# chinmay5/vit_ae_plus_plus

Measured on AMD Instinct MI355X. Metric: pretrain volumes/sec (96^3x4ch, mask 0.75) at 1/2/4/8 MI355X + recon-loss parity, higher is better.
Workload: dtype bf16; 1 GPU; ViT-B/16^3 contrastive MAE full optimisation step (fwd+loss+bwd+grad-norm+AdamW), synthetic BraTS-shape 96^3x4ch, batch 4/GPU, mask 0.75 (BASELINE config 2); global_batch=4, parallelism=dp1, rccl_ranks=1, hip_graph=True, weights=product initialize_weights, seed 0

## Files before the change

vit_ae_plus_plus_amd/csrc/gemm_bt.hpp:

```cpp
#pragma once
#include <cstdlib>
#include <type_traits>
#include "glds_gemm.hpp"

namespace vglds {

using K0 = std::integral_constant<int, 0>; using K1 = std::integral_constant<int, 1>;
using K2 = std::integral_constant<int, 2>; using K3 = std::integral_constant<int, 3>;

__device__ __forceinline__ void wg_barrier() {
    __builtin_amdgcn_sched_barrier(0);
    __builtin_amdgcn_s_barrier();
    __builtin_amdgcn_sched_barrier(0);
}


template <int S, int PT> __device__ __forceinline__ void wait_tiles(const int fly) {
    if (S >= 5 && fly >= 3) wait_vmcnt<(S >= 5 ? 3 : 1) * PT>();
    else if (S >= 4 && fly >= 2) wait_vmcnt<(S >= 4 ? 2 : 1) * PT>();
    else if (fly >= 1) wait_vmcnt<PT>();
    else wait_vmcnt<0>();
}

static inline bool bt_k_ranges(const int K, const int min_tiles, int& splits, int& kps) {
// ... 67 lines not shown
#pragma unroll
            for (int e = 0; e < 4; ++e) v[e] += bias4[e];
            f32x4 axv = {0.f, 0.f, 0.f, 0.f};
            if (need_aux) {
                if constexpr (AUX16) {
                    const bf16x4 h = ax16[pb * LB + q];
                    axv = f32x4{(float)h[0], (float)h[1], (float)h[2], (float)h[3]};
                } else {
                    axv = ax[pb * LB + q];
                }
            }
            if (epi == VITAE_EPI_GELU) {
                f32x4 y, dy;
                if (p.exact) {
#pragma unroll
                    for (int e = 0; e < 4; ++e) { float ye, de; gelu_erf_both(v[e], ye, de); y[e] = ye; dy[e] = de; }
                } else {
                    gelu_fast4(v, y, dy);
                }
                const f32x4 sv = p.auxd ? dy : v;
                if (ok) {
                    if constexpr (AUX16) {
                        bf16x4 h;
#pragma unroll
                        for (int e = 0; e < 4; ++e) h[e] = (__bf16)sv[e];
                        *reinterpret_cast<bf16x4*>(reinterpret_cast<__bf16*>(p.aux) + m * ldaux + n) = h;
                    } else {
                        *reinterpret_cast<f32x4*>(p.aux + m * ldaux + n) = sv;
                    }
                }
                v = y;
            } else if (epi == VITAE_EPI_DGELU) {
                f32x4 g = axv;
                if (!p.auxd) {
                    if (p.exact) {
#pragma unroll
                        for (int e = 0; e < 4; ++e) g[e] = gelu_erf_grad(axv[e]);
                    } else {
                        g = gelu_fast_grad4(axv);
                    }
                }
#pragma unroll
                for (int e = 0; e < 4; ++e) v[e] *= g[e];
            } else if (epi == VITAE_EPI_RELU_MASK) {
#pragma unroll
                for (int e = 0; e < 4; ++e) v[e] = axv[e] > 0.f ? v[e] : 0.f;
            } else if (epi == VITAE_EPI_RELU) {
#pragma unroll
                for (int e = 0; e < 4; ++e) v[e] = fmaxf(v[e], 0.f);
            }
            if (has_res) {
#pragma unroll
                for (int e = 0; e < 4; ++e) v[e] += rs[pb * LB + q][e];
            }
            if (acc_c) {
#pragma unroll
                for (int e = 0; e < 4; ++e) v[e] += co[pb * LB + q][e];
            }
            if (ok) {
                if (p.C) *reinterpret_cast<f32x4*>(p.C + m * ldc + n) = v;
                if (p.C16) {
                    bf16x4 v16;
#pragma unroll
                    for (int e = 0; e < 4; ++e) v16[e] = (__bf16)v[e];
                    *reinterpret_cast<bf16x4*>(p.C16 + m * ldc16 + n) = v16;
                }
                if (p.out_colsum) {
#pragma unroll
                    for (int e = 0; e < 4; ++e) csum[e] += v[e];
                }
                if (p.sqacc) sqs += (v[0] * v[0] + v[1] * v[1]) + (v[2] * v[2] + v[3] * v[3]);
            }
        }
    }
}

__device__ __forceinline__ int bt_epilogue_kind(const GArgs& p) {
    const bool res = p.residual != nullptr, accc = p.C && p.accumulate;
    if (p.epi == VITAE_EPI_NONE) return res && accc ? 7 : res ? 1 : accc ? 2 : 0;
    if (res || accc) return 7;
    return p.epi == VITAE_EPI_GELU ? 3 : p.epi == VITAE_EPI_DGELU ? 4 : p.epi == VITAE_EPI_RELU_MASK ? 5 : p.epi == VITAE_EPI_RELU ? 6 : 7;
}

template <int FM, int FN>
__device__ __forceinline__ void bt_wave_epilogue(const GArgs& p, int kind, int mb, int nb, const float* Tw, int lane, float& sqs, const f32x4 bias4,
                                                 f32x4& csum, const bool defer_colsum) {
    constexpr int LPR = 8 * FN;
    const bool full = mb + 32 * FM <= p.M && nb + 32 * FN <= p.N;
#define VITAE_BT_ROWS(E)                                                                       \
    case E:                                                                                    \
        if (full) bt_wave_rows<FM, FN, E, true, false>(p, mb, nb, Tw, lane, sqs, csum, bias4);  \
        else bt_wave_rows<FM, FN, E, false, false>(p, mb, nb, Tw, lane, sqs, csum, bias4);      \
        break;
#define VITAE_BT_ROWS_AUX(E)                                                                   \
    case E:                                                                                    \
        if (p.aux16) {                                                                         \
            if (full) bt_wave_rows<FM, FN, E, true, true>(p, mb, nb, Tw, lane, sqs, csum, bias4);  \
            else bt_wave_rows<FM, FN, E, false, true>(p, mb, nb, Tw, lane, sqs, csum, bias4);      \
        } else {                                                                               \
            if (full) bt_wave_rows<FM, FN, E, true, false>(p, mb, nb, Tw, lane, sqs, csum, bias4); \
            else bt_wave_rows<FM, FN, E, false, false>(p, mb, nb, Tw, lane, sqs, csum, bias4);     \
        }                                                                                      \
        break;
    switch (kind) {
        VITAE_BT_ROWS(0) VITAE_BT_ROWS(1) VITAE_BT_ROWS(2) VITAE_BT_ROWS_AUX(3) VITAE_BT_ROWS_AUX(4) VITAE_BT_ROWS_AUX(5) VITAE_BT_ROWS(6)
        default:
            if (p.aux16) bt_wave_rows<FM, FN, 7, false, true>(p, mb, nb, Tw, lane, sqs, csum, bias4);
            else bt_wave_rows<FM, FN, 7, false, false>(p, mb, nb, Tw, lane, sqs, csum, bias4);
            break;
    }
#undef VITAE_BT_ROWS
#undef VITAE_BT_ROWS_AUX
    if (defer_colsum) return;
    if (p.out_colsum) {
#pragma unroll
        for (int e = 0; e < 4; ++e)
#pragma unroll
            for (int d = LPR; d < 64; d <<= 1) csum[e] += __shfl_xor(csum[e], d, 64);
        const int n = nb + 4 * (lane % LPR);
        if (lane < LPR && n < p.N) {
#pragma unroll
            for (int e = 0; e < 4; ++e) atomicAdd(p.out_colsum + n + e, csum[e]);
        }
    }
}

template <int FM, int FN, int NACC>
__device__ __forceinline__ void bt_park_quadrant(const f32x16 (&acc)[NACC][FM * FN], int lane, float* Tw) {
    constexpr int S = 32 * FN;
    const int l31 = lane & 31, hi = lane >> 5;
#pragma unroll
    for (int fm = 0; fm < FM; ++fm)
#pragma unroll
        for (int fn = 0; fn < FN; ++fn)
#pragma unroll
            for (int r = 0; r < 16; ++r) {
                float v = acc[0][fm * FN + fn][r];
                if (NACC == 2) v += acc[NACC - 1][fm * FN + fn][r];
                Tw[(fm * 32 + crow(r, hi)) * S + fn * 32 + l31] = v;
            }
}

template <int BM, int BN, int WM, int WN, int NACC, class Stamp>
__device__ __forceinline__ void bt_tail(const GArgs& p, f32x16 (&acc)[2][2][NACC][BtCfg<BM, BN, WM, WN>::FM * BtCfg<BM, BN, WM, WN>::FN],
                                        unsigned char* smem, const int m0, const int n0, const int tm, const int tn, const int zid,
                                        const int wave, const int lane, Stamp stamp) {
    using Cf = BtCfg<BM, BN, WM, WN>;
    constexpr int NW = Cf::NW, HM = Cf::HM, HN = Cf::HN, FM = Cf::FM, FN = Cf::FN, NF = FM * FN;
    const int wm = wave / WN, wn = wave % WN;
    constexpr int TW = 32 * FM * 32 * FN;
    static_assert(NW * TW * 4 + 64 <= Cf::SMEM, "wave-private staging (+ the norm share of each wave) fits the operand stages");
    float* Tw = reinterpret_cast<float*>(smem) + wave * TW;
    float sqs = 0.f;
    const int kind = bt_epilogue_kind(p);
    if constexpr (BM * BN < 256 * 256) if (p.splits > 1) {
        constexpr int NT = 64 * NW, GROUPS = 4 * NF * 4;
        const int tile = p.tile0 + tm * p.tiles_n + tn;
        float* part = p.ws + VITAE_GLDS_TICKETS + (long)tile * p.splits * (NT * GROUPS * 4);
        const __amdgpu_buffer_rsrc_t rs = __builtin_amdgcn_make_buffer_rsrc(part, 0, p.splits * (NT * GROUPS * 16), 0x00020000);
        typedef unsigned u32x4 __attribute__((ext_vector_type(4)));
        const int toff = (int)threadIdx.x * 16;
        if constexpr (NACC == 2) {
#pragma unroll
            for (int a = 0; a < 2; ++a)
#pragma unroll
                for (int b = 0; b < 2; ++b)
#pragma unroll
                    for (int f = 0; f < NF; ++f)
#pragma unroll
                        for (int i = 0; i < 16; ++i) acc[a][b][0][f][i] += acc[a][b][NACC - 1][f][i];
        }
#pragma unroll
        for (int a = 0; a < 2; ++a)
#pragma unroll
            for (int b = 0; b < 2; ++b)
#pragma unroll
                for (int f = 0; f < NF; ++f)
#pragma unroll
                    for (int g = 0; g < 4; ++g) {
                        f32x4 v;
#pragma unroll
                        for (int e = 0; e < 4; ++e) v[e] = acc[a][b][0][f][4 * g + e];
                        const int grp = ((a * 2 + b) * NF + f) * 4 + g;
                        __builtin_amdgcn_raw_buffer_store_b128(__builtin_bit_cast(u32x4, v), rs, (zid * GROUPS + grp) * (NT * 16) + toff, 0, 16);
// ... 140 lines not shown
```

vit_ae_plus_plus_amd/csrc/gemm_glds.hip:

```cpp
#include <cstdlib>
#include "common.hpp"
#include "glds_tiles.hpp"
#include "glds_gemm.hpp"
#include "vitae_hip.h"

namespace {

using namespace vglds;

long long* g_gemm_dbg = nullptr;
double* g_wgrad_sqacc = nullptr;
int g_wgrad_sq_mask = 0, g_wgrad_sq_stride = 0;
static inline void set_sq(vglds::GArgs& p) { p.sqacc = g_wgrad_sqacc; p.sq_mask = g_wgrad_sq_mask; p.sq_stride = g_wgrad_sq_stride; }

struct EpiPre { f32x4 bias, res[4]; bool have; };

template <int BM, int BN, int NW>
__device__ __forceinline__ void epilogue_prefetch(const GArgs& p, int m0, int n0, EpiPre& e) {
    constexpr int NT = 64 * NW, CG = BN / 4, RPP = NT / CG, PASSES = BM / RPP;
    e.have = false;
    if constexpr (BM == 64 && BN == 64 && NW == 4) {
        static_assert(PASSES == 4, "prefetch geometry");
        if (!p.vec_epi) return;
        e.have = true;
// ... 462 lines not shown
    if (wave == 0 && n < N) {
        const f32x4 t = (red[0][lane] + red[1][lane]) + (red[2][lane] + red[3][lane]);
#pragma unroll
        for (int e = 0; e < 4; ++e) atomicAdd(out + n + e, t[e]);
    }
}

inline void launch_colsum_bf16(const void* dy16, float* out, int M, int N, hipStream_t st) {
    const int gx = cdiv(N, 256);
    constexpr int tgt = 320;
    int rpw = cdiv(cdiv(M, cdiv(tgt, gx)), 4);
    if (rpw < 4) rpw = 4;
    hipLaunchKernelGGL(colsum_bf16_kernel, dim3(gx, cdiv(M, 4 * rpw)), dim3(256), 0, st, reinterpret_cast<const __bf16*>(dy16), out, M, N, rpw);
}

struct Tile { int bm, bn, id; };

inline int vec_epilogue_ok(const GArgs& p) {
    if (p.N & 3) return 0;
    auto ok = [](const void* ptr, long ld, int align) { return !ptr || (!(ld & 3) && !((uintptr_t)ptr & (align - 1))); };
    return ok(p.C, p.ldc, 16) && ok(p.C16, p.ldc16, 8) && ok(p.aux, p.ldaux, 16) && ok(p.residual, p.ldr, 16) && ok(p.bias, 0, 16);
}

inline int xcd_by_rows(int M, int N) { return M > N; }

inline Tile pick_tile(int M, int N) {
    constexpr int wide_min = 400;
    if (N >= 128 && (long)cdiv(M, 64) * cdiv(N, 128) >= wide_min) return {64, 128, 1};
    return {64, 64, 0};
}

int g_bt_mode = env_int("VITAE_BT_TILE", -1);

struct BtPlan { int tile, split; double clocks; };

inline int old_split_rule(int M, int N, int K) {
    constexpr int min_kt = 8, target = 384;
    const Tile t = pick_tile(M, N);
    const long tiles = (long)cdiv(M, t.bm) * cdiv(N, t.bn);
    if (tiles >= target / 2 || tiles > VITAE_GLDS_TICKETS) return 1;
    long s = (target + tiles - 1) / tiles;
    const long max_by_k = K / (BK * min_kt);
    if (s > max_by_k) s = max_by_k;
    if (s > 32) s = 32;
    return s < 1 ? 1 : (int)s;
}

inline double est_64row(int M, int N, int K, bool allow_split, bool wgrad_form) {
    const Tile t = pick_tile(M, N);
    const int s = allow_split ? old_split_rule(M, N, K) : 1;
    const double nk = (double)K / BK / s, wgs = (double)cdiv(M, t.bm) * cdiv(N, t.bn) * s;
    const double c = t.id == 1 ? 3800 + 1250 * nk : 5100 + (wgrad_form ? 650 : 400) * nk;
    const double lat = 8000 + (t.id == 1 ? 1000 : 760) * nk + (s > 1 ? 7000 : 0);
    const double thr = wgs * c / 256;
    return thr > lat ? thr : lat;
}

inline BtPlan bt_plan(int M, int N, int K, int a_kc, int b_kc, bool allow_split, long cap = -1, bool allow_ws64 = true, int only = -1) {
    BtPlan best{-1, 1, 1e30};
    if (g_bt_mode == -2 || K < 2 * BK || (K % BK) || (!a_kc && b_kc) || (N & 3)) return best;
    const int nkt = K / BK;
    constexpr double ws_kt = 800.0;
    constexpr int ws_min_rows = 2048;
    constexpr int ws_min_rows_fwd = 800;
    constexpr int ws_long_k = 8192;
    constexpr double ws_kt_w = 900.0;
    constexpr double ws_fix = 14000.0;
    constexpr double ws64_kt_w = 650.0;
    constexpr double bt_fix0 = 9000.0, bt_fix1 = 4000.0;
    constexpr double wsw_kt = 1350.0;
    for (int id : {0, 3, 4, 5, 6, 7}) {
        if (only >= 0 && id != only) continue;
        if (id == 7 && g_bt_mode != 7 && only != 7) continue;
        if (id == 6 && (a_kc || b_kc)) continue;
        if (id == 5 && g_bt_mode != 5 && !allow_ws64) continue;
        if (g_bt_mode >= 0 && id != g_bt_mode) continue;
        if (id == 4 && g_bt_mode < 0 && (a_kc ? M : K) < ((a_kc && b_kc) ? ws_min_rows_fwd : ws_min_rows) && K < ws_long_k) continue;
        if (id == 6 && g_bt_mode < 0 && K < ws_min_rows && K < ws_long_k && (long)M * N < (1L << 22)) continue;
        int bm, bn;
        bt_tile_dims(id, bm, bn);
        const bool forced = g_bt_mode >= 0;
        if (!forced && (M < bm / 2 || N < bn / 2)) continue;
        const long tiles = (long)cdiv(M, bm) * cdiv(N, bn);
        const int fsplit = ENV_INT_ONCE("VITAE_BT_SPLIT", 0);
        for (int s = 1; s <= (id >= 3 && allow_split ? (id == 6 ? 4 : 8) : 1); ++s) {
            if (forced && fsplit > 0 && s != fsplit) continue;
            const int kps = cdiv(cdiv(K, s), BK) * BK;
            if (cdiv(K, kps) != s || kps < (forced ? 2 : 4) * BK || K - (s - 1) * kps < 2 * BK) continue;
            if (s > 1 && (tiles > VITAE_GLDS_TICKETS || (cap >= 0 && VITAE_GLDS_TICKETS + tiles * s * bm * bn > cap))) continue;
            const double wgs = (double)tiles * s, slots = id == 3 ? 512 : 256;
            const double rounds = (double)cdiv((long)wgs, (long)slots);
            const double nk = (double)nkt / s;
            const double per = id == 0 ? 3000 + ((!a_kc && !b_kc) ? 4300 : 2950) * nk + 14500
                             : id == 6 ? ws_fix + 4000 + wsw_kt * nk + (s > 1 ? 9000 + 4000 * s : 0)
                             : id == 4 ? ws_fix + ((!a_kc && !b_kc) ? ws_kt_w : ws_kt) * nk + (s > 1 ? 6000 + 2200 * s : 0)
                                       : 4500 + 1800 * nk + 7500 + (s > 1 ? bt_fix0 + bt_fix1 * s : 0);
            double clk = rounds * per;
            if (id == 7) {
                const double over = wgs > 256 ? (wgs - 256) / 256 : 0, kt = ((!a_kc && !b_kc && wgs >= 512) ? ws64_kt_w : 420) * 1.5;
                const double lat = (7500 + kt * nk + (s > 1 ? 3000 + 1000 * s : 0)) * (1 + 0.2 * over), thr = wgs * (4000 + kt * nk) / 256;
                clk = lat > thr ? lat : thr;
                if (nkt >= 128) clk *= 1.25;
            }
            if (id == 5) {
                const double over = wgs > 256 ? (wgs - 256) / 256 : 0, kt64 = (!a_kc && !b_kc && wgs >= 512) ? ws64_kt_w : 420;
                const double lat = (6500 + kt64 * nk + (s > 1 ? 3000 + 1000 * s : 0)) * (1 + 0.2 * over), thr = wgs * (3000 + kt64 * nk) / 256;
                clk = lat > thr ? lat : thr;
                if (nkt >= 128) clk *= 1.25;
            }
            if (clk < best.clocks) best = BtPlan{id, s, clk};
        }
    }
    if (best.tile < 0 || g_bt_mode >= 0 || only >= 0) return best;
    if (best.clocks >= 0.92 * est_64row(M, N, K, allow_split, !a_kc && !b_kc) * (nkt >= 128 ? 1.25 : 1.0)) return BtPlan{-1, 1, 0.0};
    return best;
}

template <int BM1, int BN1>
void launch_pair(int id2, dim3 grid, hipStream_t st, const GArgs& p1, const GArgs& p2, int nb1) {
    dim3 block(256);
    if (id2 == 0) hipLaunchKernelGGL((gemm_glds_pair_kernel<BM1, BN1, 64, 64>), grid, block, 0, st, p1, p2, nb1);
    else hipLaunchKernelGGL((gemm_glds_pair_kernel<BM1, BN1, 64, 128>), grid, block, 0, st, p1, p2, nb1);
}

}

extern "C" int vitae_gemm_glds_set_bt_tile(int mode) {
    if (mode < -2 || mode > 7 || mode == 1 || mode == 2) return VITAE_ERR_INVALID_ARG;
    g_bt_mode = mode;
    return VITAE_OK;
}

extern "C" int vitae_gemm_glds_bt_choice(int a_kcontig, int b_kcontig, int M, int N, int K) { return bt_plan(M, N, K, a_kcontig, b_kcontig, true).tile; }

extern "C" int vitae_gemm_glds_pick_split_k(int M, int N, int K) {
    const BtPlan bp = bt_plan(M, N, K, 1, 1, true);
    if (bp.tile >= 0) return bp.split;
    return old_split_rule(M, N, K);
}

extern "C" int vitae_gemm_glds_pick_split_k_form(int a_kcontig, int b_kcontig, int M, int N, int K) {
    const BtPlan bp = bt_plan(M, N, K, a_kcontig, b_kcontig, true);
    if (bp.tile >= 0) return bp.split;
    return old_split_rule(M, N, K);
}

extern "C" long vitae_gemm_glds_ws_floats(int M, int N, int split_k) {
    if (split_k <= 1) return 0;
    const Tile t = pick_tile(M, N);
    const long small = (long)cdiv(M, t.bm) * cdiv(N, t.bn) * t.bm * t.bn, big = (long)cdiv(M, 128) * cdiv(N, 128) * 128 * 128;
    const long wide = (long)cdiv(M, 128) * cdiv(N, 256) * 128 * 256;
    long m = small > big ? small : big;
    if (wide > m) m = wide;
    return VITAE_GLDS_TICKETS + m * split_k;
}

static int gemm_glds_launch(int a_kcontig, int b_kcontig, const void* A16, long lda, const void* B16, long ldb,
                            float* C, long ldc, void* C16, long ldc16, int M, int N, int K, const float* bias,
                            const float* residual, long ldr, int epi, float* aux, long ldaux, int accumulate,
                            int split_k, float* splitk_ws, float* out_colsum_accum, void* stream,
                            const BtPlan* forced = nullptr) {
    if (!A16 || !B16 || (!C && !C16) || M <= 0 || N <= 0 || K <= 0) return VITAE_ERR_INVALID_ARG;
    const int aux16 = (epi & VITAE_EPI_AUX_BF16) != 0, auxd = (epi & VITAE_EPI_AUX_DERIV) != 0;
    epi &= ~(VITAE_EPI_AUX_BF16 | VITAE_EPI_AUX_DERIV);
    if (epi != VITAE_EPI_NONE && epi != VITAE_EPI_RELU && !aux) return VITAE_ERR_INVALID_ARG;
    if (auxd && epi != VITAE_EPI_GELU && epi != VITAE_EPI_DGELU) return VITAE_ERR_INVALID_ARG;
    if (K % BK) return VITAE_ERR_UNSUPPORTED_SHAPE;
    if ((long)M * (ldc > N ? ldc : N) >= (1L << 31) || (long)M * ldaux >= (1L << 31) || (long)M * ldr >= (1L << 31) ||
        (long)M * ldc16 >= (1L << 31))
// ... 367 lines not shown
```

vit_ae_plus_plus_amd/csrc/gemm_ws64.hip:

```cpp
#include "gemm_bt.hpp"

namespace vglds {

#ifndef VITAE_WS64_STAGES
#define VITAE_WS64_STAGES 4
#endif
constexpr int WS64_SMEM = VITAE_WS64_STAGES * 16384;
template <bool A_KC, bool B_KC, int S, bool RS, bool W2 = false, int BM = 64>
__device__ __forceinline__ void gemm_ws64_body(const GArgs& p, const WsHot& h, const int bid, const int zid, unsigned char* smem) {
#ifndef VITAE_WS64_PRODUCERS
#define VITAE_WS64_PRODUCERS 4
#endif
    constexpr int BN = 64, NWC = 4, NWP = VITAE_WS64_PRODUCERS, FM = BM / 64;
    static_assert(BM == 64 || (BM == 128 && !W2), "64 or 128 rows");
    constexpr int A_T = BM * BK * 2, B_T = BN * BK * 2, STG = A_T + (W2 ? 2 : 1) * B_T;
    constexpr int PA = pieces<BM, A_KC, NWP>(), PB = pieces<BN, B_KC, NWP>(), PT = PA + (W2 ? 2 : 1) * PB;
    static_assert(!W2 || (A_KC && B_KC && !RS), "two weight planes: the forward form");
    static_assert(S >= 3 && S <= 5 && (S - 2) * PT <= 63, "stage count");
    const int T = h.tiles_m * h.tiles_n;
    const int xq = T >> 3, xr = T & 7, xcd = bid & 7;
    const int lin = (xcd < xr ? xcd * (xq + 1) : xr * (xq + 1) + (xcd - xr) * xq) + (bid >> 3);
    if ((bid >> 3) >= xq + (xcd < xr ? 1 : 0)) return;
    const int tn = (h.xcd_m & 1) ? lin % h.tiles_n : lin / h.tiles_m;
    const int tm = (h.xcd_m & 1) ? lin / h.tiles_n : lin % h.tiles_m;
    const int m0 = tm * BM, n0 = tn * BN;
    const int kbeg = zid * h.kps;
    const int nk = (min(h.K, kbeg + h.kps) - kbeg) / BK;
    const int lane = threadIdx.x & 63;
    const int wave = __builtin_amdgcn_readfirstlane(threadIdx.x >> 6);
    auto stamp = [&](int i) {
        if ((h.xcd_m & 2) && (threadIdx.x & 255) == 0) p.dbg[((long)blockIdx.z * gridDim.x + blockIdx.x) * 16 + i] = __builtin_amdgcn_s_memtime();
    };
    if (wave >= NWC) {
        const int pw = wave - NWC;
        stamp(8);
        auto issue_tile = [&](int t, int stage) {
            unsigned char* dst = smem + stage * STG;
            const int k0 = kbeg + t * BK;
#pragma unroll
            for (int j = 0; j < PA; ++j) dma_piece<BM, A_KC, NWP>(h.A, h.lda, h.M, m0, k0, dst, pw, lane, j);
#pragma unroll
            for (int j = 0; j < PB; ++j) dma_piece<BN, B_KC, NWP>(h.B, h.ldb, h.N, n0, k0, dst + A_T, pw, lane, j);
            if constexpr (W2) {
#pragma unroll
                for (int j = 0; j < PB; ++j) dma_piece<BN, B_KC, NWP>(h.B2, h.ldb, h.N, n0, k0, dst + A_T + B_T, pw, lane, j);
            }
        };
        const int npre = min(S - 1, nk);
        for (int t = 0; t < npre; ++t) issue_tile(t, t);
        stamp(9);
        wait_tiles<S, PT>(npre - 1);
        stamp(10);
        wg_barrier();
        int stage = npre % S;
#pragma unroll 1
        for (int t = 0; t + 1 < nk; ++t) {
            if (t + S - 1 < nk) {
                issue_tile(t + S - 1, stage);
                stage = stage + 1 == S ? 0 : stage + 1;
            }
            wait_tiles<S, PT>(min(t + S - 1, nk - 1) - (t + 1));
            wg_barrier();
        }
        stamp(11);
        return;
    }
    const int wm = wave >> 1, wn = wave & 1;
    const int l31 = lane & 31, hi = lane >> 5;
    f32x16 acc[2];
#pragma unroll
    for (int h = 0; h < 2; ++h)
#pragma unroll
        for (int i = 0; i < 16; ++i) acc[h][i] = 0.f;
    const bool rowsum = RS && p.a_rowsum != nullptr && tn == 0 && wn == 0;
    f32x16 accx;
#pragma unroll
    for (int i = 0; i < 16; ++i) accx[i] = 0.f;
    bf16x8 ones;
#pragma unroll
    for (int i = 0; i < 8; ++i) ones[i] = (__bf16)1.0f;
    bf16x8 fa[FM][BK / 16], fb[BK / 16], fb2[W2 ? BK / 16 : 1];
    constexpr int RK = FM * (A_KC ? 1 : 2) + (W2 ? 2 : 1) * (B_KC ? 1 : 2);
    static_assert(2 * RK <= 15, "the counted lgkmcnt of ws64_consume");
    bf16x8 sel[2];
    if constexpr (FM == 2 && RS) {
#pragma unroll
        for (int i = 0; i < 8; ++i) {
            sel[0][i] = (__bf16)((lane & 16) ? 0.0f : 1.0f);
            sel[1][i] = (__bf16)((lane & 16) ? 1.0f : 0.0f);
        }
    }
    auto rd = [&](const unsigned char* TA, auto kk_c) {
        constexpr int kk = decltype(kk_c)::value;
        fa[0][kk] = frag_asm<BM, A_KC>(TA, wm * (BM / 2), kk, lane);
        if constexpr (FM == 2) fa[1][kk] = frag_asm<BM, A_KC>(TA, wm * (BM / 2) + 32, kk, lane);
        fb[kk] = frag_asm<BN, B_KC>(TA + A_T, wn * 32, kk, lane);
        if constexpr (W2) fb2[kk] = frag_asm<BN, B_KC>(TA + A_T + B_T, wn * 32, kk, lane);
    };
    auto mm = [&](auto kk_c) {
        constexpr int kk = decltype(kk_c)::value;
        if constexpr (FM == 2) {
            frag_tie(fa[0][kk]); frag_tie(fa[1][kk]); frag_tie(fb[kk]);
            acc[0] = __builtin_amdgcn_mfma_f32_32x32x16_bf16(fa[0][kk], fb[kk], acc[0], 0, 0, 0);
            acc[1] = __builtin_amdgcn_mfma_f32_32x32x16_bf16(fa[1][kk], fb[kk], acc[1], 0, 0, 0);
            if constexpr (RS) {
                if (rowsum) {
                    accx = __builtin_amdgcn_mfma_f32_32x32x16_bf16(sel[0], fa[0][kk], accx, 0, 0, 0);
                    accx = __builtin_amdgcn_mfma_f32_32x32x16_bf16(sel[1], fa[1][kk], accx, 0, 0, 0);
                }
            }
            return;
        }
        frag_tie(fa[0][kk]); frag_tie(fb[kk]);
        if constexpr (W2) {
            frag_tie(fb2[kk]);
            acc[kk & 1] = __builtin_amdgcn_mfma_f32_32x32x16_bf16(fa[0][kk], fb2[kk], acc[kk & 1], 0, 0, 0);
// ... 2 lines not shown
        if constexpr (RS) {
            if (rowsum) accx = __builtin_amdgcn_mfma_f32_32x32x16_bf16(fa[0][kk], ones, accx, 0, 0, 0);
        }
    };
    const int nq = n0 + wn * 32 + 4 * (lane % 8);
    f32x4 bias4 = {0.f, 0.f, 0.f, 0.f};
    if (p.bias && nq < p.N) bias4 = *reinterpret_cast<const f32x4*>(p.bias + nq);
    stamp(0);
    wg_barrier();
    stamp(1);
    ws64_consume<2 * RK, S, STG>(smem, nk, rd, mm);
    if constexpr (FM == 2) {
        if (RS && rowsum && hi == 0) {
            const int m = m0 + wm * 64 + l31;
            if (m < p.M) atomicAdd(p.a_rowsum + m, accx[0]);
            if (m + 32 < p.M) atomicAdd(p.a_rowsum + m + 32, accx[8]);
        }
    }
    if (FM == 1 && RS && rowsum && l31 == 0) {
#pragma unroll
        for (int r = 0; r < 16; ++r) {
            const int m = m0 + wm * 32 + crow(r, hi);
            if (m < p.M) atomicAdd(p.a_rowsum + m, accx[r]);
        }
    }
    stamp(2);
    f32x16 accs[1][FM];
    if constexpr (FM == 2) {
        accs[0][0] = acc[0]; accs[0][1] = acc[1];
    } else {
#pragma unroll
        for (int i = 0; i < 16; ++i) accs[0][0][i] = acc[0][i] + acc[1][i];
    }
    __syncthreads();
    float* Tw = reinterpret_cast<float*>(smem) + wave * (1024 * FM);
    if (p.splits > 1) {
        const int tile = p.tile0 + tm * p.tiles_n + tn;
        float* part = p.ws + VITAE_GLDS_TICKETS + (long)tile * p.splits * (BM * BN);
        const __amdgpu_buffer_rsrc_t rs = __builtin_amdgcn_make_buffer_rsrc(part, 0, p.splits * (BM * BN * 4), 0x00020000);
        typedef unsigned u32x4 __attribute__((ext_vector_type(4)));
        const int toff = (int)threadIdx.x * 16;
#pragma unroll
        for (int g = 0; g < 4 * FM; ++g) {
            const f32x4 v = {accs[0][g >> 2][4 * (g & 3)], accs[0][g >> 2][4 * (g & 3) + 1], accs[0][g >> 2][4 * (g & 3) + 2], accs[0][g >> 2][4 * (g & 3) + 3]};
            __builtin_amdgcn_raw_buffer_store_b128(__builtin_bit_cast(u32x4, v), rs, (zid * (4 * FM) + g) * (256 * 16) + toff, 0, 16);
        }
        asm volatile("s_waitcnt vmcnt(0)" ::: "memory");
        __syncthreads();
        int* flag = reinterpret_cast<int*>(smem + 4 * 4096 * FM);
        if (threadIdx.x == 0) *flag = __hip_atomic_fetch_add(reinterpret_cast<int*>(p.ws) + tile, 1, __ATOMIC_RELAXED, __HIP_MEMORY_SCOPE_AGENT);
        __syncthreads();
        stamp(3);
        if (*flag != p.splits - 1) return;
#pragma unroll
        for (int f = 0; f < FM; ++f)
#pragma unroll
            for (int i = 0; i < 16; ++i) accs[0][f][i] = 0.f;
        constexpr int SU = 4 / FM;
#pragma unroll 1
        for (int sp0 = 0; sp0 < p.splits; sp0 += SU) {
            f32x4 v[SU][4 * FM];
#pragma unroll
            for (int u = 0; u < SU; ++u) {
                const int sp = min(sp0 + u, p.splits - 1);
#pragma unroll
                for (int g = 0; g < 4 * FM; ++g)
                    v[u][g] = __builtin_bit_cast(f32x4, __builtin_amdgcn_raw_buffer_load_b128(rs, (sp * (4 * FM) + g) * (256 * 16) + toff, 0, 16));
            }
#pragma unroll
            for (int u = 0; u < SU; ++u)
                if (sp0 + u < p.splits) {
#pragma unroll
                    for (int g = 0; g < 4 * FM; ++g)
#pragma unroll
                        for (int e = 0; e < 4; ++e) accs[0][g >> 2][4 * (g & 3) + e] += v[u][g][e];
                }
        }
        if (threadIdx.x == 0) __hip_atomic_store(reinterpret_cast<int*>(p.ws) + tile, 0, __ATOMIC_RELAXED, __HIP_MEMORY_SCOPE_AGENT);
    }
    stamp(4);
    bt_park_quadrant<FM, 1, 1>(accs, lane, Tw);
    __builtin_amdgcn_wave_barrier();
    float sqs = 0.f;
    { f32x4 cz = {0.f, 0.f, 0.f, 0.f}; bt_wave_epilogue<FM, 1>(p, bt_epilogue_kind(p), m0 + wm * (BM / 2), n0 + wn * 32, Tw, lane, sqs, bias4, cz, false); }
    stamp(5);
    if (p.sqacc) {
        sqs = wave_sum(sqs);
        float* red = reinterpret_cast<float*>(smem + 4 * 4096 * FM + 64);
        if (lane == 0) red[wave] = sqs;
        __syncthreads();
        if (threadIdx.x == 0) atomicAdd(sq_slot(p), (double)((red[0] + red[1]) + (red[2] + red[3])));
    }
    if (p.dbg) { asm volatile("s_waitcnt vmcnt(0)" ::: "memory"); stamp(6); }
}

template <bool A_KC, bool B_KC>
__global__ __launch_bounds__(64 * (4 + VITAE_WS64_PRODUCERS), 2) void gemm_ws64_kernel(WS_HOT_PARAMS, const GArgs p) {
    __shared__ __attribute__((aligned(1024))) unsigned char smem[WS64_SMEM];
    const WsHot h = WS_HOT_FROM_PARAMS;
    gemm_ws64_body<A_KC, B_KC, VITAE_WS64_STAGES, false>(p, h, blockIdx.x, blockIdx.z, smem);
}

constexpr int WS128X64_STAGES = 3, WS128X64_SMEM = WS128X64_STAGES * 24576;
template <bool A_KC, bool B_KC>
__global__ __launch_bounds__(64 * (4 + VITAE_WS64_PRODUCERS), 2) void gemm_ws64_m128_kernel(WS_HOT_PARAMS, const GArgs p) {
    __shared__ __attribute__((aligned(1024))) unsigned char smem[WS128X64_SMEM];
    const WsHot h{A, B, B2, lda, ldb, M, N, K, (M + 127) >> 7, (N + 63) >> 6, xcd_m, kps};
    gemm_ws64_body<A_KC, B_KC, WS128X64_STAGES, false, false, 128>(p, h, blockIdx.x, blockIdx.z, smem);
}

void ws64_launch(const GArgs& p, int a_kc, int b_kc, int id, hipStream_t st) {
    const dim3 grid(8 * cdiv((long)p.tiles_m * p.tiles_n, 8), 1, p.splits), block(64 * (4 + VITAE_WS64_PRODUCERS));
    if (id == 7) {
        if (a_kc && b_kc) hipLaunchKernelGGL((gemm_ws64_m128_kernel<true, true>), grid, block, 0, st, WS_HOT_ARGS(p), p);
        else if (a_kc && !b_kc) hipLaunchKernelGGL((gemm_ws64_m128_kernel<true, false>), grid, block, 0, st, WS_HOT_ARGS(p), p);
        else hipLaunchKernelGGL((gemm_ws64_m128_kernel<false, false>), grid, block, 0, st, WS_HOT_ARGS(p), p);
        return;
    }
    if (a_kc && b_kc) hipLaunchKernelGGL((gemm_ws64_kernel<true, true>), grid, block, 0, st, WS_HOT_ARGS(p), p);
    else if (a_kc && !b_kc) hipLaunchKernelGGL((gemm_ws64_kernel<true, false>), grid, block, 0, st, WS_HOT_ARGS(p), p);
    else hipLaunchKernelGGL((gemm_ws64_kernel<false, false>), grid, block, 0, st, WS_HOT_ARGS(p), p);
}

constexpr int WS64W2_STAGES = 3;
__global__ __launch_bounds__(64 * (4 + VITAE_WS64_PRODUCERS), 2) void gemm_ws64_w2_kernel(WS_HOT_PARAMS, const GArgs p) {
    __shared__ __attribute__((aligned(1024))) unsigned char smem[WS64W2_STAGES * 24576];
    gemm_ws64_body<true, true, WS64W2_STAGES, false, true>(p, WS_HOT_FROM_PARAMS, blockIdx.x, blockIdx.z, smem);
}

int ws64_w2_launch(GArgs p, hipStream_t st) {
    if (!p.vec_epi || !p.B2 || p.a_rowsum || (p.K % BK) || p.splits < 1) return VITAE_ERR_UNSUPPORTED_SHAPE;
    if (!bt_k_ranges(p.K, 2, p.splits, p.k_per_split)) return VITAE_ERR_UNSUPPORTED_SHAPE;
    p.tiles_m = cdiv(p.M, 64); p.tiles_n = cdiv(p.N, 64); p.tile0 = 0;
    if (p.splits > 1 && (!p.ws || (long)p.tiles_m * p.tiles_n > VITAE_GLDS_TICKETS || p.epi == VITAE_EPI_GELU)) return VITAE_ERR_UNSUPPORTED_SHAPE;
    const dim3 grid(8 * cdiv((long)p.tiles_m * p.tiles_n, 8), 1, p.splits), block(64 * (4 + VITAE_WS64_PRODUCERS));
    hipLaunchKernelGGL(gemm_ws64_w2_kernel, grid, block, 0, st, WS_HOT_ARGS(p), p);
    return vitae_launch_status();
}

template <bool RS, int BM1, int BM2>
__global__ __launch_bounds__(64 * (4 + VITAE_WS64_PRODUCERS), 2) void gemm_ws64_pair_kernel(const __bf16* A, const __bf16* B1, const __bf16* B2, int lda, int ldb,
                                                                                           int M1, int N1, int K1, int K2, int kps1, int packed,
                                                                                           const GArgs p1, const GArgs p2) {
    constexpr int S1 = BM1 == 128 ? WS128X64_STAGES : VITAE_WS64_STAGES, S2 = BM2 == 128 ? WS128X64_STAGES : VITAE_WS64_STAGES;
    constexpr int SMEM = (BM1 == 128 || BM2 == 128) ? WS128X64_SMEM : WS64_SMEM;
    static_assert(SMEM >= WS64_SMEM && 2 * SMEM <= 160 * 1024, "either body's stages; two workgroups per CU");
    __shared__ __attribute__((aligned(1024))) unsigned char smem[SMEM];
    const int nb1 = packed & 0xfffff, splits1 = (packed >> 20) & 15, dbg2 = (packed >> 25) & 2;
    if ((int)blockIdx.x < nb1 * splits1) {
        const WsHot h{A, B1, nullptr, lda, ldb, M1, N1, K1, (M1 + BM1 - 1) >> (BM1 == 128 ? 7 : 6), (N1 + 63) >> 6, ((packed >> 24) & 1) | dbg2, kps1};
        gemm_ws64_body<true, false, S1, false, false, BM1>(p1, h, blockIdx.x % nb1, blockIdx.x / nb1, smem);
    } else {
        const WsHot h{A, B2, nullptr, lda, ldb, K1, N1, K2, (K1 + BM2 - 1) >> (BM2 == 128 ? 7 : 6), (N1 + 63) >> 6, ((packed >> 25) & 1) | dbg2, K2};
        gemm_ws64_body<false, false, S2, RS, false, BM2>(p2, h, blockIdx.x - nb1 * splits1, 0, smem);
    }
}

template <bool RS>
static void ws64_pair_dispatch(int bm1, int bm2, dim3 grid, dim3 block, hipStream_t st, const GArgs& p1, const GArgs& p2, int packed) {
#define VITAE_WS64_PAIR(B1, B2)                                                                                                              \
    hipLaunchKernelGGL((gemm_ws64_pair_kernel<RS, B1, B2>), grid, block, 0, st, p1.A, p1.B, p2.B, (int)p1.lda, (int)p1.ldb, p1.M, p1.N, p1.K, \
                       p2.K, p1.k_per_split, packed, p1, p2)
    if (bm1 == 64 && bm2 == 64) VITAE_WS64_PAIR(64, 64);
    else if (bm1 == 64) VITAE_WS64_PAIR(64, 128);
    else if (bm2 == 64) VITAE_WS64_PAIR(128, 64);
    else VITAE_WS64_PAIR(128, 128);
#undef VITAE_WS64_PAIR
}

int ws64_pair_launch(GArgs p1, GArgs p2, hipStream_t st, int bm1, int bm2) {
    if ((bm1 != 64 && bm1 != 128) || (bm2 != 64 && bm2 != 128)) return VITAE_ERR_INVALID_ARG;
    if (!p1.vec_epi || !p2.vec_epi || (p1.K % BK) || (p2.K % BK) || p2.K < 2 * BK || p1.a_rowsum) return VITAE_ERR_UNSUPPORTED_SHAPE;
    if (p1.splits < 1) p1.splits = 1;
    if (!bt_k_ranges(p1.K, 2, p1.splits, p1.k_per_split)) return VITAE_ERR_UNSUPPORTED_SHAPE;
    p1.tiles_m = cdiv(p1.M, bm1); p1.tiles_n = cdiv(p1.N, 64); p1.tile0 = 0;
    p2.tiles_m = cdiv(p2.M, bm2); p2.tiles_n = cdiv(p2.N, 64); p2.tile0 = 0;
    p2.k_per_split = p2.K; p2.splits = 1;
    if (p1.splits > 1 && (!p1.ws || (long)p1.tiles_m * p1.tiles_n > VITAE_GLDS_TICKETS)) return VITAE_ERR_UNSUPPORTED_SHAPE;
    const int nb1 = 8 * cdiv((long)p1.tiles_m * p1.tiles_n, 8), nb2 = 8 * cdiv((long)p2.tiles_m * p2.tiles_n, 8);
    const dim3 grid(nb1 * p1.splits + nb2), block(64 * (4 + VITAE_WS64_PRODUCERS));
    if (p1.A != p2.A || p1.lda != p2.lda || p1.ldb != p2.ldb || p2.M != p1.K || p2.N != p1.N || nb1 >= (1 << 20) || p1.splits > 15 ||
        p1.lda >= (1L << 31) || p1.ldb >= (1L << 31)) return VITAE_ERR_UNSUPPORTED_SHAPE;
    const int packed = nb1 | p1.splits << 20 | (p1.xcd_m & 1) << 24 | (p2.xcd_m & 1) << 25 | ((p1.dbg || p2.dbg) ? 1 << 26 : 0);
    if (p2.a_rowsum) ws64_pair_dispatch<true>(bm1, bm2, grid, block, st, p1, p2, packed);
    else ws64_pair_dispatch<false>(bm1, bm2, grid, block, st, p1, p2, packed);
    return vitae_launch_status();
}

}
```

Measured before the change: 1153 volumes/s.

## Specialize ws64 epilogue kinds per GEMM role and merge pair kernel variants

Adds a compile-time mask of allowed epilogue kinds so forward, dgrad and wgrad ws64 kernels only instantiate the epilogue paths they can use; unsupported kinds fall back to the generic path. The pair kernel drops its template variants: tile-size choice moves into runtime bits of the packed argument. The pair kernel also splits into producer-wave and consumer-wave code paths through a ROLE parameter. The aim is to cut code size and register pressure from unused epilogue instantiations, at the cost of runtime branching and always reserving the larger shared-memory buffer in the pair kernel. The rowsum template flag is now fixed to true for the pair's second GEMM.

```diff
diff --git a/vit_ae_plus_plus_amd/csrc/gemm_bt.hpp b/vit_ae_plus_plus_amd/csrc/gemm_bt.hpp
--- a/vit_ae_plus_plus_amd/csrc/gemm_bt.hpp
+++ b/vit_ae_plus_plus_amd/csrc/gemm_bt.hpp
@@ -173,24 +173,41 @@
     return p.epi == VITAE_EPI_GELU ? 3 : p.epi == VITAE_EPI_DGELU ? 4 : p.epi == VITAE_EPI_RELU_MASK ? 5 : p.epi == VITAE_EPI_RELU ? 6 : 7;
 }
 
-template <int FM, int FN>
+constexpr int bt_kind(int k) { return 1 << k; }
+constexpr int bt_kind16(int k) { return 1 << (8 + k); }
+constexpr int BT_KINDS_ALL = 0x7f | bt_kind16(3) | bt_kind16(4) | bt_kind16(5);
+constexpr int BT_KINDS_FWD = BT_KINDS_ALL & ~(bt_kind(4) | bt_kind16(4) | bt_kind(5) | bt_kind16(5));
+constexpr int BT_KINDS_DGRAD = bt_kind(0) | bt_kind(2) | bt_kind(4) | bt_kind16(4);
+constexpr int BT_KINDS_WGRAD = bt_kind(0) | bt_kind(2);
+
+template <int FM, int FN, int KINDS = BT_KINDS_ALL>
 __device__ __forceinline__ void bt_wave_epilogue(const GArgs& p, int kind, int mb, int nb, const float* Tw, int lane, float& sqs, const f32x4 bias4,
                                                  f32x4& csum, const bool defer_colsum) {
     constexpr int LPR = 8 * FN;
     const bool full = mb + 32 * FM <= p.M && nb + 32 * FN <= p.N;
+    if constexpr (KINDS != BT_KINDS_ALL) {
+        const int bit = kind + ((kind >= 3 && kind <= 5 && p.aux16) ? 8 : 0);
+        if (kind > 6 || !((KINDS >> bit) & 1)) kind = 7;
+    }
 #define VITAE_BT_ROWS(E)                                                                       \
     case E:                                                                                    \
-        if (full) bt_wave_rows<FM, FN, E, true, false>(p, mb, nb, Tw, lane, sqs, csum, bias4);  \
-        else bt_wave_rows<FM, FN, E, false, false>(p, mb, nb, Tw, lane, sqs, csum, bias4);      \
+        if constexpr ((KINDS & bt_kind(E)) != 0) {                                             \
+            if (full) bt_wave_rows<FM, FN, E, true, false>(p, mb, nb, Tw, lane, sqs, csum, bias4);  \
+            else bt_wave_rows<FM, FN, E, false, false>(p, mb, nb, Tw, lane, sqs, csum, bias4);      \
+        }                                                                                      \
         break;
 #define VITAE_BT_ROWS_AUX(E)                                                                   \
     case E:                                                                                    \
         if (p.aux16) {                                                                         \
-            if (full) bt_wave_rows<FM, FN, E, true, true>(p, mb, nb, Tw, lane, sqs, csum, bias4);  \
-            else bt_wave_rows<FM, FN, E, false, true>(p, mb, nb, Tw, lane, sqs, csum, bias4);      \
+            if constexpr ((KINDS & bt_kind16(E)) != 0) {                                       \
+                if (full) bt_wave_rows<FM, FN, E, true, true>(p, mb, nb, Tw, lane, sqs, csum, bias4);  \
+                else bt_wave_rows<FM, FN, E, false, true>(p, mb, nb, Tw, lane, sqs, csum, bias4);      \
+            }                                                                                  \
         } else {                                                                               \
-            if (full) bt_wave_rows<FM, FN, E, true, false>(p, mb, nb, Tw, lane, sqs, csum, bias4); \
-            else bt_wave_rows<FM, FN, E, false, false>(p, mb, nb, Tw, lane, sqs, csum, bias4);     \
+            if constexpr ((KINDS & bt_kind(E)) != 0) {                                         \
+                if (full) bt_wave_rows<FM, FN, E, true, false>(p, mb, nb, Tw, lane, sqs, csum, bias4); \
+                else bt_wave_rows<FM, FN, E, false, false>(p, mb, nb, Tw, lane, sqs, csum, bias4);     \
+            }                                                                                  \
         }                                                                                      \
         break;
     switch (kind) {
diff --git a/vit_ae_plus_plus_amd/csrc/gemm_glds.hip b/vit_ae_plus_plus_amd/csrc/gemm_glds.hip
--- a/vit_ae_plus_plus_amd/csrc/gemm_glds.hip
+++ b/vit_ae_plus_plus_amd/csrc/gemm_glds.hip
@@ -568,9 +568,9 @@
         const bool forced = g_bt_mode >= 0;
         if (!forced && (M < bm / 2 || N < bn / 2)) continue;
         const long tiles = (long)cdiv(M, bm) * cdiv(N, bn);
-        const int fsplit = ENV_INT_ONCE("VITAE_BT_SPLIT", 0);
+        const int fsplit = forced && allow_split ? env_int("VITAE_BT_SPLIT", 0) : 0;
         for (int s = 1; s <= (id >= 3 && allow_split ? (id == 6 ? 4 : 8) : 1); ++s) {
-            if (forced && fsplit > 0 && s != fsplit) continue;
+            if (fsplit > 0 && s != fsplit) continue;
             const int kps = cdiv(cdiv(K, s), BK) * BK;
             if (cdiv(K, kps) != s || kps < (forced ? 2 : 4) * BK || K - (s - 1) * kps < 2 * BK) continue;
             if (s > 1 && (tiles > VITAE_GLDS_TICKETS || (cap >= 0 && VITAE_GLDS_TICKETS + tiles * s * bm * bn > cap))) continue;
diff --git a/vit_ae_plus_plus_amd/csrc/gemm_ws64.hip b/vit_ae_plus_plus_amd/csrc/gemm_ws64.hip
--- a/vit_ae_plus_plus_amd/csrc/gemm_ws64.hip
+++ b/vit_ae_plus_plus_amd/csrc/gemm_ws64.hip
@@ -6,7 +6,7 @@
 #define VITAE_WS64_STAGES 4
 #endif
 constexpr int WS64_SMEM = VITAE_WS64_STAGES * 16384;
-template <bool A_KC, bool B_KC, int S, bool RS, bool W2 = false, int BM = 64>
+template <bool A_KC, bool B_KC, int S, bool RS, bool W2 = false, int BM = 64, int KINDS = BT_KINDS_ALL, int ROLE = 0>
 __device__ __forceinline__ void gemm_ws64_body(const GArgs& p, const WsHot& h, const int bid, const int zid, unsigned char* smem) {
 #ifndef VITAE_WS64_PRODUCERS
 #define VITAE_WS64_PRODUCERS 4
@@ -31,7 +31,7 @@
     auto stamp = [&](int i) {
         if ((h.xcd_m & 2) && (threadIdx.x & 255) == 0) p.dbg[((long)blockIdx.z * gridDim.x + blockIdx.x) * 16 + i] = __builtin_amdgcn_s_memtime();
     };
-    if (wave >= NWC) {
+    if (ROLE != 2 && (ROLE == 1 || wave >= NWC)) {
         const int pw = wave - NWC;
         stamp(8);
         auto issue_tile = [&](int t, int stage) {
@@ -200,7 +200,7 @@
     bt_park_quadrant<FM, 1, 1>(accs, lane, Tw);
     __builtin_amdgcn_wave_barrier();
     float sqs = 0.f;
-    { f32x4 cz = {0.f, 0.f, 0.f, 0.f}; bt_wave_epilogue<FM, 1>(p, bt_epilogue_kind(p), m0 + wm * (BM / 2), n0 + wn * 32, Tw, lane, sqs, bias4, cz, false); }
+    { f32x4 cz = {0.f, 0.f, 0.f, 0.f}; bt_wave_epilogue<FM, 1, KINDS>(p, bt_epilogue_kind(p), m0 + wm * (BM / 2), n0 + wn * 32, Tw, lane, sqs, bias4, cz, false); }
     stamp(5);
     if (p.sqacc) {
         sqs = wave_sum(sqs);
@@ -212,11 +212,13 @@
     if (p.dbg) { asm volatile("s_waitcnt vmcnt(0)" ::: "memory"); stamp(6); }
 }
 
+template <bool A_KC, bool B_KC> constexpr int ws64_kinds() { return A_KC && B_KC ? BT_KINDS_FWD : A_KC ? BT_KINDS_DGRAD : BT_KINDS_WGRAD; }
+
 template <bool A_KC, bool B_KC>
 __global__ __launch_bounds__(64 * (4 + VITAE_WS64_PRODUCERS), 2) void gemm_ws64_kernel(WS_HOT_PARAMS, const GArgs p) {
     __shared__ __attribute__((aligned(1024))) unsigned char smem[WS64_SMEM];
     const WsHot h = WS_HOT_FROM_PARAMS;
-    gemm_ws64_body<A_KC, B_KC, VITAE_WS64_STAGES, false>(p, h, blockIdx.x, blockIdx.z, smem);
+    gemm_ws64_body<A_KC, B_KC, VITAE_WS64_STAGES, false, false, 64, ws64_kinds<A_KC, B_KC>()>(p, h, blockIdx.x, blockIdx.z, smem);
 }
 
 constexpr int WS128X64_STAGES = 3, WS128X64_SMEM = WS128X64_STAGES * 24576;
@@ -224,7 +226,7 @@
 __global__ __launch_bounds__(64 * (4 + VITAE_WS64_PRODUCERS), 2) void gemm_ws64_m128_kernel(WS_HOT_PARAMS, const GArgs p) {
     __shared__ __attribute__((aligned(1024))) unsigned char smem[WS128X64_SMEM];
     const WsHot h{A, B, B2, lda, ldb, M, N, K, (M + 127) >> 7, (N + 63) >> 6, xcd_m, kps};
-    gemm_ws64_body<A_KC, B_KC, WS128X64_STAGES, false, false, 128>(p, h, blockIdx.x, blockIdx.z, smem);
+    gemm_ws64_body<A_KC, B_KC, WS128X64_STAGES, false, false, 128, ws64_kinds<A_KC, B_KC>()>(p, h, blockIdx.x, blockIdx.z, smem);
 }
 
 void ws64_launch(const GArgs& p, int a_kc, int b_kc, int id, hipStream_t st) {
@@ -243,7 +245,7 @@
 constexpr int WS64W2_STAGES = 3;
 __global__ __launch_bounds__(64 * (4 + VITAE_WS64_PRODUCERS), 2) void gemm_ws64_w2_kernel(WS_HOT_PARAMS, const GArgs p) {
     __shared__ __attribute__((aligned(1024))) unsigned char smem[WS64W2_STAGES * 24576];
-    gemm_ws64_body<true, true, WS64W2_STAGES, false, true>(p, WS_HOT_FROM_PARAMS, blockIdx.x, blockIdx.z, smem);
+    gemm_ws64_body<true, true, WS64W2_STAGES, false, true, 64, BT_KINDS_FWD>(p, WS_HOT_FROM_PARAMS, blockIdx.x, blockIdx.z, smem);
 }
 
 int ws64_w2_launch(GArgs p, hipStream_t st) {
@@ -256,34 +258,36 @@
     return vitae_launch_status();
 }
 
-template <bool RS, int BM1, int BM2>
 __global__ __launch_bounds__(64 * (4 + VITAE_WS64_PRODUCERS), 2) void gemm_ws64_pair_kernel(const __bf16* A, const __bf16* B1, const __bf16* B2, int lda, int ldb,
                                                                                            int M1, int N1, int K1, int K2, int kps1, int packed,
                                                                                            const GArgs p1, const GArgs p2) {
-    constexpr int S1 = BM1 == 128 ? WS128X64_STAGES : VITAE_WS64_STAGES, S2 = BM2 == 128 ? WS128X64_STAGES : VITAE_WS64_STAGES;
-    constexpr int SMEM = (BM1 == 128 || BM2 == 128) ? WS128X64_SMEM : WS64_SMEM;
-    static_assert(SMEM >= WS64_SMEM && 2 * SMEM <= 160 * 1024, "either body's stages; two workgroups per CU");
-    __shared__ __attribute__((aligned(1024))) unsigned char smem[SMEM];
+    static_assert(WS128X64_SMEM >= WS64_SMEM && 2 * WS128X64_SMEM <= 160 * 1024, "either body's stages; two workgroups per CU");
+    __shared__ __attribute__((aligned(1024))) unsigned char smem[WS128X64_SMEM];
     const int nb1 = packed & 0xfffff, splits1 = (packed >> 20) & 15, dbg2 = (packed >> 25) & 2;
-    if ((int)blockIdx.x < nb1 * splits1) {
-        const WsHot h{A, B1, nullptr, lda, ldb, M1, N1, K1, (M1 + BM1 - 1) >> (BM1 == 128 ? 7 : 6), (N1 + 63) >> 6, ((packed >> 24) & 1) | dbg2, kps1};
-        gemm_ws64_body<true, false, S1, false, false, BM1>(p1, h, blockIdx.x % nb1, blockIdx.x / nb1, smem);
+#define VITAE_WS64_PAIR_HALVES(ROLE)                                                                                                              \
+    if ((int)blockIdx.x < nb1 * splits1) {                                                                                                        \
+        if ((packed >> 27) & 1) {                                                                                                                 \
+            const WsHot h{A, B1, nullptr, lda, ldb, M1, N1, K1, (M1 + 127) >> 7, (N1 + 63) >> 6, ((packed >> 24) & 1) | dbg2, kps1};             \
+            gemm_ws64_body<true, false, WS128X64_STAGES, false, false, 128, BT_KINDS_DGRAD, ROLE>(p1, h, blockIdx.x % nb1, blockIdx.x / nb1, smem); \
+        } else {                                                                                                                                  \
+            const WsHot h{A, B1, nullptr, lda, ldb, M1, N1, K1, (M1 + 63) >> 6, (N1 + 63) >> 6, ((packed >> 24) & 1) | dbg2, kps1};              \
+            gemm_ws64_body<true, false, VITAE_WS64_STAGES, false, false, 64, BT_KINDS_DGRAD, ROLE>(p1, h, blockIdx.x % nb1, blockIdx.x / nb1, smem); \
+        }                                                                                                                                         \
+    } else {                                                                                                                                      \
+        if ((packed >> 28) & 1) {                                                                                                                 \
+            const WsHot h{A, B2, nullptr, lda, ldb, K1, N1, K2, (K1 + 127) >> 7, (N1 + 63) >> 6, ((packed >> 25) & 1) | dbg2, K2};               \
+            gemm_ws64_body<false, false, WS128X64_STAGES, true, false, 128, BT_KINDS_WGRAD, ROLE>(p2, h, blockIdx.x - nb1 * splits1, 0, smem);    \
+        } else {                                                                                                                                  \
+            const WsHot h{A, B2, nullptr, lda, ldb, K1, N1, K2, (K1 + 63) >> 6, (N1 + 63) >> 6, ((packed >> 25) & 1) | dbg2, K2};                \
+            gemm_ws64_body<false, false, VITAE_WS64_STAGES, true, false, 64, BT_KINDS_WGRAD, ROLE>(p2, h, blockIdx.x - nb1 * splits1, 0, smem);   \
+        }                                                                                                                                         \
+    }
+    if (__builtin_amdgcn_readfirstlane(threadIdx.x >> 6) >= 4) {
+        VITAE_WS64_PAIR_HALVES(1)
     } else {
-        const WsHot h{A, B2, nullptr, lda, ldb, K1, N1, K2, (K1 + BM2 - 1) >> (BM2 == 128 ? 7 : 6), (N1 + 63) >> 6, ((packed >> 25) & 1) | dbg2, K2};
-        gemm_ws64_body<false, false, S2, RS, false, BM2>(p2, h, blockIdx.x - nb1 * splits1, 0, smem);
-    }
-}
-
-template <bool RS>
-static void ws64_pair_dispatch(int bm1, int bm2, dim3 grid, dim3 block, hipStream_t st, const GArgs& p1, const GArgs& p2, int packed) {
-#define VITAE_WS64_PAIR(B1, B2)                                                                                                              \
-    hipLaunchKernelGGL((gemm_ws64_pair_kernel<RS, B1, B2>), grid, block, 0, st, p1.A, p1.B, p2.B, (int)p1.lda, (int)p1.ldb, p1.M, p1.N, p1.K, \
-                       p2.K, p1.k_per_split, packed, p1, p2)
-    if (bm1 == 64 && bm2 == 64) VITAE_WS64_PAIR(64, 64);
-    else if (bm1 == 64) VITAE_WS64_PAIR(64, 128);
-    else if (bm2 == 64) VITAE_WS64_PAIR(128, 64);
-    else VITAE_WS64_PAIR(128, 128);
-#undef VITAE_WS64_PAIR
+        VITAE_WS64_PAIR_HALVES(2)
+    }
+#undef VITAE_WS64_PAIR_HALVES
 }
 
 int ws64_pair_launch(GArgs p1, GArgs p2, hipStream_t st, int bm1, int bm2) {
@@ -299,9 +303,10 @@
     const dim3 grid(nb1 * p1.splits + nb2), block(64 * (4 + VITAE_WS64_PRODUCERS));
     if (p1.A != p2.A || p1.lda != p2.lda || p1.ldb != p2.ldb || p2.M != p1.K || p2.N != p1.N || nb1 >= (1 << 20) || p1.splits > 15 ||
         p1.lda >= (1L << 31) || p1.ldb >= (1L << 31)) return VITAE_ERR_UNSUPPORTED_SHAPE;
-    const int packed = nb1 | p1.splits << 20 | (p1.xcd_m & 1) << 24 | (p2.xcd_m & 1) << 25 | ((p1.dbg || p2.dbg) ? 1 << 26 : 0);
-    if (p2.a_rowsum) ws64_pair_dispatch<true>(bm1, bm2, grid, block, st, p1, p2, packed);
-    else ws64_pair_dispatch<false>(bm1, bm2, grid, block, st, p1, p2, packed);
+    const int packed = nb1 | p1.splits << 20 | (p1.xcd_m & 1) << 24 | (p2.xcd_m & 1) << 25 | ((p1.dbg || p2.dbg) ? 1 << 26 : 0) |
+                       (bm1 == 128 ? 1 << 27 : 0) | (bm2 == 128 ? 1 << 28 : 0);
+    hipLaunchKernelGGL(gemm_ws64_pair_kernel, grid, block, 0, st, p1.A, p1.B, p2.B, (int)p1.lda, (int)p1.ldb, p1.M, p1.N, p1.K, p2.K, p1.k_per_split,
+                       packed, p1, p2);
     return vitae_launch_status();
 }
 
```

Result: faster. 1171 volumes/s, median of 6 (+1.5%).
